# JaronTu/Multimodal_MVD_Seg

Hardware: AMD Instinct MI355X
Metric: train-step samples/sec on 4-modality 128^3 patches (PlainConvUNet 3d_fullres, fp32) (higher is better)
Workload: dtype f32; 1 GPU; BASELINE configs[1]: PlainConvUNet 3d_fullres 6 stages 31.2M params, 4x128x128x128 patch, 5 classes, fp32, DC+CE deep supervision, SGD-Nesterov+clip; per_gpu_batch=2, global_batch=2, parallelism=dp1, step_launch=one hipGraph replay per step (captured after 3 eager steps)

## Files before the change

multimodal_mvd_seg_amd/csrc/conv_mfma.hip:

```cpp
#include <stdlib.h>
#include <type_traits>

#include "common.h"
#include "conv_geom.h"

namespace mvd {

typedef float f32x16 __attribute__((ext_vector_type(16)));

struct FwdTile {
    int ED, EH, EW, nslots;
    int min_off[3];
    int ntd, nth, ntw;
    int K;
    int toff[27];
    int dbg;
};

__device__ __forceinline__ void store_tile32(const FwdGeom &g, const f32x16 &acc, float bv, int n, int od, int ohb, int ow0,
                                             int k, int hh, int S, int split, int Ktot, float *__restrict__ part,
                                             float *__restrict__ y1, float *__restrict__ y2) {
    const int owl = ow0 + 4 * hh;
    if (S > 1) {
        float *pl = part + (size_t)(4 * hh) * Ktot + k;
// ... 360 lines not shown
        if (c0 < g.C1) {
            src = a1; Cs = g.C1; cofs = c0;
        } else {
            src = a2; Cs = g.C2; cofs = c0 - g.C1;
        }
        load_w(cc, 0);
        __syncthreads();
        for (int base = 0; base < XR; base += XB) {
            float4 v[XB];
#pragma unroll
            for (int u = 0; u < XB; u++) {
                const int idx = (base + u) * 256 + tid;
                v[u] = make_float4(0.f, 0.f, 0.f, 0.f);
                if (base + u < XR && idx < nx && !(tg.dbg & 1)) {
                    const int slot = idx >> 3;
                    const int ez = (slot * tg.magHW) >> 16, rem = slot - ez * EHW;
                    const int ey = (rem * tg.magW) >> 16, ex = rem - ey * tg.EW;
                    const int id = iz0 + ez, ih = iy0 + ey, iw = ix0 + ex;
                    if (id >= 0 && id < g.Di && ih >= 0 && ih < g.Hi && iw >= 0 && iw < g.Wi)
                        v[u] = *reinterpret_cast<const float4 *>(
                            src + ((((size_t)n * g.Di + id) * g.Hi + ih) * g.Wi + iw) * Cs + cofs + (tid & 7) * 4);
                }
            }
#pragma unroll
            for (int u = 0; u < XB; u++) {
                const int idx = (base + u) * 256 + tid;
                if (base + u < XR) *reinterpret_cast<float4 *>(Xs + (size_t)(idx >> 3) * XS + (idx & 7) * 4) = v[u];
            }
        }
        for (int gi = 0; gi < ngroups; gi++) {
            store_w(gi & 1);
            __syncthreads();
            if (gi + 1 < ngroups) load_w(cc, gi + 1);
            if (!(tg.dbg & 2)) {
                const float *wb_ = Wsm + (size_t)(gi & 1) * WBUF;
#pragma unroll
                for (int tl = 0; tl < TG; tl++) {
                    const int t = gi * TG + tl;
                    if (t < g.ntaps) {
                        const int to = __builtin_amdgcn_readlane(toff_l, t);
                        float4 af[MT][4], bf[NT][4];
#pragma unroll
                        for (int m = 0; m < MT; m++) {
                            const float4 *pa = reinterpret_cast<const float4 *>(Xs + (size_t)(sbase[m] + to) * XS + h * 16);
#pragma unroll
                            for (int e = 0; e < 4; e++) af[m][e] = pa[e];
                        }
#pragma unroll
                        for (int q = 0; q < NT; q++) {
                            const float4 *pb = reinterpret_cast<const float4 *>(wb_ + ((size_t)(tl * 2 + h) * KT + q * 32 + i) * WS);
#pragma unroll
                            for (int e = 0; e < 4; e++) bf[q][e] = pb[e];
                        }
#pragma unroll
                        for (int e = 0; e < 4; e++) {
#pragma unroll
                            for (int c4 = 0; c4 < 4; c4++)
#pragma unroll
                                for (int m = 0; m < MT; m++)
#pragma unroll
                                    for (int q = 0; q < NT; q++) {
                                        const float avv = c4 == 0 ? af[m][e].x : (c4 == 1 ? af[m][e].y : (c4 == 2 ? af[m][e].z : af[m][e].w));
                                        const float bvv = c4 == 0 ? bf[q][e].x : (c4 == 1 ? bf[q][e].y : (c4 == 2 ? bf[q][e].z : bf[q][e].w));
                                        acc[m][q] = __builtin_amdgcn_mfma_f32_32x32x2f32(avv, bvv, acc[m][q], 0, 0, 0);
                                    }
                        }
                    }
                }
            }
        }
    }
    const int od = od0 + wave;
    if (od >= g.Do) return;
#pragma unroll
    for (int m = 0; m < MT; m++)
#pragma unroll
        for (int q = 0; q < NT; q++) {
            const int k = kb * KT + q * 32 + i;
            const float bv = settled((bias && tg.S == 1) ? bias[k] : 0.f);
            store_tile32(g, acc[m][q], bv, n, od, oh0 + 4 * m, ow0, k, h, tg.S, split, tg.K, part, y1, y2);
        }
}

constexpr int SXR = 12;
constexpr int SXB = 6;
__global__ __launch_bounds__(512, 1) void k_fwd32s(const FwdGeom g, const Fwd32Tile tg, const float *__restrict__ a1,
                                                   const float *__restrict__ a2, const float *__restrict__ w,
                                                   const float *__restrict__ bias, float *__restrict__ y1,
                                                   float *__restrict__ y2, float *__restrict__ stats) {
    extern __shared__ __attribute__((aligned(16))) float Xs[];
    constexpr int XS = 36;
    const int tid = threadIdx.x, lane = tid & 63;
    const int wave = __builtin_amdgcn_readfirstlane(tid >> 6);
    const int i = lane & 31, h = lane >> 5;
    const int per_xcd = (tg.nitems + 7) >> 3;
    const int item = (int)(blockIdx.x & 7) * per_xcd + (int)(blockIdx.x >> 3);
    if (item >= tg.nitems) return;
    unsigned r_ = (unsigned)item;
    const int kb = (int)(r_ % (unsigned)tg.nkb); r_ /= (unsigned)tg.nkb;
    const int tw_ = (int)(r_ % (unsigned)tg.ntw); r_ /= (unsigned)tg.ntw;
    const int th_ = (int)(r_ % (unsigned)tg.nth); r_ /= (unsigned)tg.nth;
    const int td_ = (int)(r_ % (unsigned)tg.ntd);
    const int n = (int)(r_ / (unsigned)tg.ntd);

    const int C = g.C1 + g.C2;
    const int nch = C >> 5;
    const int EHW = tg.EH * tg.EW;
    const int nx = tg.nslots * 8;
    const int od0 = td_ * 2, oh0 = th_ * 4, ow0 = tw_ * 8;
    const int iz0 = od0 * 2 + tg.min_off[0], iy0 = oh0 * 2 + tg.min_off[1], ix0 = ow0 * 2 + tg.min_off[2];
    const int dl = wave & 1, kh = (wave >> 1) & 1, tap_half = wave >> 2;
    const int tb = tap_half ? 14 : 0, nt = tap_half ? g.ntaps - 14 : 14;
    const int sbase = ((2 * dl) * tg.EH + 2 * (i >> 3)) * tg.EW + 2 * (i & 7);
    const float4 *xlane = reinterpret_cast<const float4 *>(Xs + (size_t)sbase * XS + h * 16);
    const int kcol = kb * 64 + kh * 32 + i;
    const float *wlane = w + (((size_t)h * tg.K + kcol) << 4);
    const size_t wtap = (size_t)2 * tg.K * 16;

    const bool fastst = tg.EH == 9 && tg.EW == 17 && tg.nslots == 765;
    const int r3 = tid / 136, rem = tid - r3 * 136;
    const int sx = rem >> 3, part = rem & 7;
    const bool st_act = tid < 408;
    const int iw = ix0 + sx;
    const bool okw = st_act && iw >= 0 && iw < g.Wi;
    bool okr[3];
#pragma unroll
    for (int v = 0; v < 3; v++) {
        const int ih = iy0 + r3 + 3 * v;
        okr[v] = okw && ih >= 0 && ih < g.Hi;
    }
    float4 *lds_st = reinterpret_cast<float4 *>(Xs + (size_t)(r3 * 17 + sx) * XS + part * 4);

    f32x16 acc;
#pragma unroll
    for (int r = 0; r < 16; r++) acc[r] = 0.f;
    const int lt = lane < g.ntaps ? lane : g.ntaps - 1;
    const int toff_l = tg.toff[lt < 27 ? lt : 26], wt_l = g.wt[lt < 27 ? lt : 26];

    for (int cc = 0; cc < nch; cc++) {
        const int c0 = cc * 32;
        const float *src;
        int Cs, cofs;
        if (c0 < g.C1) {
            src = a1; Cs = g.C1; cofs = c0;
        } else {
            src = a2; Cs = g.C2; cofs = c0 - g.C1;
        }
        const float *wc = wlane + (size_t)cc * g.T * wtap;
        float4 wb[4][4];
#pragma unroll
        for (int u = 0; u < 3; u++)
#pragma unroll
            for (int e = 0; e < 4; e++)
                wb[u][e] = *reinterpret_cast<const float4 *>(wc + (size_t)__builtin_amdgcn_readlane(wt_l, tb + u) * wtap + e * 4);
        __syncthreads();
        if (fastst) {
            const unsigned off0 = (unsigned)(((iy0 + r3) * g.Wi + iw) * Cs + cofs + part * 4) << 2;
            const unsigned drow = (unsigned)(3 * g.Wi * Cs) << 2;
            float4 v[15];
#pragma unroll
            for (int pl = 0; pl < 5; pl++) {
                const int id = iz0 + pl;
                const bool inpl = id >= 0 && id < g.Di;
                const float *plane = src + ((size_t)n * g.Di + (inpl ? id : 0)) * g.Hi * g.Wi * Cs;
                const __amdgpu_buffer_rsrc_t rp =
                    __builtin_amdgcn_make_buffer_rsrc(const_cast<float *>(plane), 0, inpl ? 0x7fffffff : 0, 0x00020000);
#pragma unroll
                for (int r = 0; r < 3; r++) {
                    const unsigned o = okr[r] ? off0 + (unsigned)r * drow : 0xffffffffu;
                    v[pl * 3 + r] = __builtin_bit_cast(float4, __builtin_amdgcn_raw_buffer_load_b128(rp, (int)o, 0, 0));
                }
            }
#pragma unroll
            for (int pq = 0; pq < 15; pq++)
                if (st_act) lds_st[((pq / 3) * 9 + 3 * (pq % 3)) * 17 * (XS / 4)] = v[pq];
        } else {
            int tid_ = tid;
            asm volatile("" : "+v"(tid_));
            for (int base = 0; base < SXR; base += SXB) {
                float4 v[SXB];
#pragma unroll
                for (int q = 0; q < SXB; q++) {
                    const int idx = (base + q) * 512 + tid_;
                    v[q] = make_float4(0.f, 0.f, 0.f, 0.f);
                    if (idx < nx) {
                        const int slot = idx >> 3;
                        const int ez = slot / EHW, rem2 = slot - ez * EHW;
                        const int ey = (rem2 * tg.magW) >> 16, ex = rem2 - ey * tg.EW;
                        const int id = iz0 + ez, ih = iy0 + ey, iw2 = ix0 + ex;
                        if (id >= 0 && id < g.Di && ih >= 0 && ih < g.Hi && iw2 >= 0 && iw2 < g.Wi)
                            v[q] = *reinterpret_cast<const float4 *>(
                                src + ((((size_t)n * g.Di + id) * g.Hi + ih) * g.Wi + iw2) * Cs + cofs + (tid_ & 7) * 4);
                    }
                }
#pragma unroll
                for (int q = 0; q < SXB; q++) {
                    const int idx = (base + q) * 512 + tid_;
                    if (idx < nx) *reinterpret_cast<float4 *>(Xs + (size_t)(idx >> 3) * XS + (idx & 7) * 4) = v[q];
                }
            }
        }
        __syncthreads();
        float4 af[2][4];
        {
            const float4 *pa = xlane + (size_t)__builtin_amdgcn_readlane(toff_l, tb) * (XS / 4);
#pragma unroll
            for (int e = 0; e < 4; e++) af[0][e] = pa[e];
        }
        for (int s0 = 0; s0 < nt; s0 += 4) {
#pragma unroll
            for (int u = 0; u < 4; u++) {
                const int sidx = s0 + u;
                if (sidx < nt) {
                    const int t = tb + sidx;
                    const int tn = sidx + 3 < nt ? t + 3 : tb + nt - 1;
#pragma unroll
                    for (int e = 0; e < 4; e++)
                        wb[(u + 3) & 3][e] =
                            *reinterpret_cast<const float4 *>(wc + (size_t)__builtin_amdgcn_readlane(wt_l, tn) * wtap + e * 4);
                    const float4 *pa = xlane + (size_t)__builtin_amdgcn_readlane(toff_l, sidx + 1 < nt ? t + 1 : tb + nt - 1) * (XS / 4);
#pragma unroll
                    for (int e = 0; e < 4; e++) af[(u + 1) & 1][e] = pa[e];
#pragma unroll
                    for (int e = 0; e < 4; e++) {
                        acc = __builtin_amdgcn_mfma_f32_32x32x2f32(af[u & 1][e].x, wb[u][e].x, acc, 0, 0, 0);
                        acc = __builtin_amdgcn_mfma_f32_32x32x2f32(af[u & 1][e].y, wb[u][e].y, acc, 0, 0, 0);
                        acc = __builtin_amdgcn_mfma_f32_32x32x2f32(af[u & 1][e].z, wb[u][e].z, acc, 0, 0, 0);
                        acc = __builtin_amdgcn_mfma_f32_32x32x2f32(af[u & 1][e].w, wb[u][e].w, acc, 0, 0, 0);
                    }
                    __builtin_amdgcn_sched_barrier(0);
                }
            }
        }
    }
    __syncthreads();
    if (tap_half) {
        float *xo = Xs + (size_t)(wave & 3) * 1024 + lane;
#pragma unroll
        for (int r = 0; r < 16; r++) xo[r * 64] = acc[r];
    }
    __syncthreads();
    if (tap_half) return;
    {
        const float *xi = Xs + (size_t)wave * 1024 + lane;
#pragma unroll
        for (int r = 0; r < 16; r++) acc[r] += xi[r * 64];
    }
    const int od = od0 + dl;
    const float bv = settled(bias ? bias[kcol] : 0.f);
    if (stats) {
        const size_t tl = ((size_t)(td_ * 2 + dl) * tg.nth + th_) * tg.ntw + tw_;
        float *so = stats + (((size_t)n * tg.ntd * 2 * tg.nth * tg.ntw + tl) * tg.K) * 2;
        float sa = 0.f, sq = 0.f;
        if (od < g.Do) {
#pragma unroll
            for (int r = 0; r < 16; r++) {
                const int row = (r & 3) + 8 * (r >> 2) + 4 * h;
                const int oh = oh0 + (row >> 3), ow = ow0 + (row & 7);
                if (oh < g.Ho && ow < g.Wo) {
                    const float val = acc[r] + bv;
                    sa += val;
                    sq += val * val;
                }
            }
        }
        sa += __shfl_xor(sa, 32);
        sq += __shfl_xor(sq, 32);
        if (h == 0) *reinterpret_cast<float2 *>(so + (size_t)kcol * 2) = make_float2(sa, sq);
    }
    if (od >= g.Do) return;
#pragma unroll
    for (int r = 0; r < 16; r++) {
        const int row = (r & 3) + 8 * (r >> 2) + 4 * h;
        const int oh = oh0 + (row >> 3), ow = ow0 + (row & 7);
        if (oh < g.Ho && ow < g.Wo) {
            const size_t ov = (((size_t)n * g.Dy + od) * g.Hy + oh) * g.Wy + ow;
            const float val = acc[r] + bv;
            if (kcol < g.K1)
                y1[ov * g.K1 + kcol] = val;
            else
                y2[ov * g.K2 + (kcol - g.K1)] = val;
        }
    }
}

struct Dg2Tile {
    int ntd, nth, ntw, ncb, nitems, C;
    int acc;
};
__global__ __launch_bounds__(512, 2) void k_dgrad32s(const FwdGeom g, const Dg2Tile tg, const float *__restrict__ dy,
                                                     const float *__restrict__ wb, float *__restrict__ dx) {
    __shared__ __attribute__((aligned(16))) float Xs[135 * 36];
    constexpr int XS = 36;
    const int tid = threadIdx.x, lane = tid & 63;
    const int wave = __builtin_amdgcn_readfirstlane(tid >> 6);
    const int i = lane & 31, h = lane >> 5;
    const int per_xcd = (tg.nitems + 7) >> 3;
    const int item = (int)(blockIdx.x & 7) * per_xcd + (int)(blockIdx.x >> 3);
    if (item >= tg.nitems) return;
    unsigned r_ = (unsigned)item;
    const int cb = (int)(r_ % (unsigned)tg.ncb); r_ /= (unsigned)tg.ncb;
    const int tw_ = (int)(r_ % (unsigned)tg.ntw); r_ /= (unsigned)tg.ntw;
    const int th_ = (int)(r_ % (unsigned)tg.nth); r_ /= (unsigned)tg.nth;
    const int td_ = (int)(r_ % (unsigned)tg.ntd);
    const int n = (int)(r_ / (unsigned)tg.ntd);
    const int K = g.C1, C = tg.C;
    const int nch = K >> 5;
    const int oz0 = td_ * 2, oy0 = th_ * 4, ox0 = tw_ * 8;
    const int ccol = cb * 32 + i;
    const float *wlane = wb + (((size_t)h * C + ccol) << 4);
    const size_t wtap = (size_t)2 * C * 16;

    f32x16 acc[2];
#pragma unroll
    for (int m = 0; m < 2; m++)
#pragma unroll
        for (int r = 0; r < 16; r++) acc[m][r] = 0.f;

    for (int kk = 0; kk < nch; kk++) {
        __syncthreads();
        {
            const __amdgpu_buffer_rsrc_t rdy = __builtin_amdgcn_make_buffer_rsrc(
                const_cast<float *>(dy + (size_t)n * g.Di * g.Hi * g.Wi * K + kk * 32), 0, 0x7fffffff, 0x00020000);
            float4 v[3];
#pragma unroll
            for (int u = 0; u < 3; u++) {
                const int idx = tid + u * 512;
                const int slot = idx >> 3, part = idx & 7;
                const int ez = slot / 45, rem = slot - ez * 45;
                const int ey = rem / 9, ex = rem - ey * 9;
                const int oz = oz0 + ez, oy = oy0 + ey, ox = ox0 + ex;
                const bool ok = idx < 135 * 8 && oz < g.Di && oy < g.Hi && ox < g.Wi;
                const unsigned o = ok ? (unsigned)(((oz * g.Hi + oy) * g.Wi + ox) * K + part * 4) * 4u : 0xffffffffu;
                v[u] = __builtin_bit_cast(float4, __builtin_amdgcn_raw_buffer_load_b128(rdy, (int)o, 0, 0));
            }
#pragma unroll
            for (int u = 0; u < 3; u++) {
                const int idx = tid + u * 512;
                if (idx < 135 * 8) *reinterpret_cast<float4 *>(Xs + (size_t)(idx >> 3) * XS + (idx & 7) * 4) = v[u];
            }
        }
        __syncthreads();
        const float *wc = wlane + (size_t)kk * 27 * wtap;
#pragma unroll
        for (int m = 0; m < 2; m++) {
            const int q = m ? 7 - wave : wave;
            const int pz = q >> 2, py = (q >> 1) & 1, px = q & 1;
            const float4 *xm = reinterpret_cast<const float4 *>(Xs + (size_t)((m * 5 + (i >> 3)) * 9 + (i & 7)) * XS + h * 16);
            const int ntq = 1 << (pz + py + px);
            auto tap_of = [&](int j, int &t, int &so) {
                const int bz = pz ? (j >> (py + px)) & 1 : 0, by = py ? (j >> px) & 1 : 0, bx = px ? j & 1 : 0;
                const int tz = pz ? (bz ? 2 : 0) : 1, ty = py ? (by ? 2 : 0) : 1, tx = px ? (bx ? 2 : 0) : 1;
                const int dz = (pz && !bz) ? 1 : 0, dyy = (py && !by) ? 1 : 0, dxx = (px && !bx) ? 1 : 0;
                t = (tz * 3 + ty) * 3 + tx;
                so = (dz * 5 + dyy) * 9 + dxx;
            };
            float4 wv[2][4];
            int t0, so0;
            tap_of(0, t0, so0);
#pragma unroll
            for (int e = 0; e < 4; e++) wv[0][e] = *reinterpret_cast<const float4 *>(wc + (size_t)t0 * wtap + e * 4);
            for (int j = 0; j < ntq; j += 2) {
#pragma unroll
                for (int u = 0; u < 2; u++) {
                    if (j + u < ntq) {
                        int t, so, tn, son;
                        tap_of(j + u, t, so);
                        tap_of(j + u + 1 < ntq ? j + u + 1 : j + u, tn, son);
#pragma unroll
                        for (int e = 0; e < 4; e++)
                            wv[(u + 1) & 1][e] = *reinterpret_cast<const float4 *>(wc + (size_t)tn * wtap + e * 4);
                        float4 af[4];
#pragma unroll
                        for (int e = 0; e < 4; e++) af[e] = xm[so * (XS / 4) + e];
#pragma unroll
                        for (int e = 0; e < 4; e++) {
                            acc[m] = __builtin_amdgcn_mfma_f32_32x32x2f32(af[e].x, wv[u][e].x, acc[m], 0, 0, 0);
                            acc[m] = __builtin_amdgcn_mfma_f32_32x32x2f32(af[e].y, wv[u][e].y, acc[m], 0, 0, 0);
                            acc[m] = __builtin_amdgcn_mfma_f32_32x32x2f32(af[e].z, wv[u][e].z, acc[m], 0, 0, 0);
                            acc[m] = __builtin_amdgcn_mfma_f32_32x32x2f32(af[e].w, wv[u][e].w, acc[m], 0, 0, 0);
                        }
                    }
                }
            }
        }
    }
    float *xl = dx + (size_t)(2 * 4 * h) * C + ccol;
#pragma unroll
    for (int m = 0; m < 2; m++) {
        const int q = m ? 7 - wave : wave;
        const int pz = q >> 2, py = (q >> 1) & 1, px = q & 1;
        const int iz = 2 * (oz0 + m) + pz;
#pragma unroll
        for (int r = 0; r < 16; r++) {
            const int iy = 2 * (oy0 + (r >> 2)) + py, ixu = 2 * (ox0 + (r & 3)) + px;
            const size_t uo = ((((size_t)n * g.Dy + iz) * g.Hy + iy) * g.Wy + ixu) * C;
            if (iz < g.Dy && iy < g.Hy && ixu + 8 * h < g.Wy) xl[uo] = tg.acc ? xl[uo] + acc[m][r] : acc[m][r];
        }
    }
}

int dgrad32s(int N, int D, int H, int W, int C, int K, int Do, int Ho, int Wo, const float *dy, const float *wb, float *dx,
             hipStream_t s, int accumulate) {
    if (C % 32 || K % 32 || (((uintptr_t)dy | (uintptr_t)wb) & 15)) return -1;
    if ((long)Do * Ho * Wo * K * 4 >= (1L << 31)) return -1;
    FwdGeom g;
    memset(&g, 0, sizeof(g));
    g.N = N;
    g.Di = Do; g.Hi = Ho; g.Wi = Wo;
    g.Dy = D; g.Hy = H; g.Wy = W;
    g.C1 = K;
    Dg2Tile tg;
    tg.ntd = (Do + 1) / 2; tg.nth = (Ho + 3) / 4; tg.ntw = (Wo + 7) / 8;
    tg.ncb = C / 32;
    tg.C = C;
    tg.acc = accumulate;
    const long nitems = (long)N * tg.ntd * tg.nth * tg.ntw * tg.ncb;
    if (nitems > (1L << 30)) return -1;
    tg.nitems = (int)nitems;
    const unsigned grid = (unsigned)(((nitems + 7) / 8) * 8);
    hipLaunchKernelGGL(k_dgrad32s, dim3(grid), dim3(512), 0, s, g, tg, dy, wb, dx);
    return check_launch("conv dgrad (stride 2, fused parity classes)");
}

static int num_cus();
static int launch_fwd32s(const FwdGeom &g, const float *a1, const float *a2, const float *w, const float *bias, float *y1,
                         float *y2, hipStream_t s, float *stats, long stats_tiles, int *stats_done, long *plan) {
    const int K = g.K1 + g.K2;
    Fwd32Tile tg;
    memset(&tg, 0, sizeof(tg));
    int mn[3] = {127, 127, 127}, mx[3] = {-127, -127, -127};
    for (int t = 0; t < g.ntaps; t++)
        for (int a = 0; a < 3; a++) {
            if (g.off[t][a] < mn[a]) mn[a] = g.off[t][a];
            if (g.off[t][a] > mx[a]) mx[a] = g.off[t][a];
        }
    const int T3[3] = {2, 4, 8};
    int E[3];
    for (int a = 0; a < 3; a++) {
        E[a] = (T3[a] - 1) * 2 + (mx[a] - mn[a]) + 1;
        tg.min_off[a] = mn[a];
    }
    tg.EH = E[1]; tg.EW = E[2];
    tg.nslots = E[0] * E[1] * E[2];
    if (tg.nslots > SXR * 64 || g.ntaps != 27) return -1;
    int m = (1 << 16) / tg.EW + 1;
    for (int nn = 0; nn < tg.EH * tg.EW; nn++)
        if (((nn * m) >> 16) != nn / tg.EW) return -1;
    tg.magW = m;
    for (int t = 0; t < g.ntaps; t++)
        tg.toff[t] = ((g.off[t][0] - mn[0]) * tg.EH + (g.off[t][1] - mn[1])) * tg.EW + (g.off[t][2] - mn[2]);
    tg.ntd = (g.Do + 1) / 2;
    tg.nth = (g.Ho + 3) / 4;
    tg.ntw = (g.Wo + 7) / 8;
    tg.nkb = K / 64;
    tg.K = K;
    const long nitems = (long)g.N * tg.ntd * tg.nth * tg.ntw * tg.nkb;
    if (nitems > (1L << 30)) return -1;
    tg.nitems = (int)nitems;
    const long my_tiles = (long)tg.ntd * 2 * tg.nth * tg.ntw;
    if (plan) {
        *plan = my_tiles;
        return 0;
    }
    float *st = (stats && stats_done && stats_tiles == my_tiles) ? stats : nullptr;
    const size_t lds = (size_t)tg.nslots * 36 * sizeof(float);
    static PerDeviceFlag cfgd;
    if (!cfgd()) {
        if (hipFuncSetAttribute(reinterpret_cast<const void *>(k_fwd32s), hipFuncAttributeMaxDynamicSharedMemorySize,
                                (int)LDS_LIMIT) != hipSuccess) {
            set_error("conv fwd (stride 2): cannot raise the dynamic LDS limit");
            return 1;
        }
        cfgd() = true;
    }
    const unsigned grid = (unsigned)(((nitems + 7) / 8) * 8);
    hipLaunchKernelGGL(k_fwd32s, dim3(grid), dim3(512), lds, s, g, tg, a1, a2, w, bias, y1, y2, st);
    if (check_launch("conv fwd (stride 2, CK=32)")) return 1;
    if (st) *stats_done = 1;
    return 0;
}

static int num_cus() {
    static int n = 0;
    if (!n) {
        hipDeviceProp_t p;
        int dev = 0;
        if (hipGetDevice(&dev) == hipSuccess && hipGetDeviceProperties(&p, dev) == hipSuccess) n = p.multiProcessorCount;
        if (n <= 0) n = 256;
    }
    return n;
}

static int split_for(const void *ws, size_t ws_bytes, long wgs, int nch, size_t out_elems, int nkb) {
    int S = 1;
    if (ws && wgs < 256 && nch >= 4) {
        long want = 512 / wgs;
        if (want > MAX_SPLIT) want = MAX_SPLIT;
        if (want > nch / 2) want = nch / 2;
        while (want > 1 && (size_t)want * out_elems * sizeof(float) > ws_bytes) want--;
        if (want > 1 && (long)nkb * want <= 65535) S = (int)want;
    }
    return S;
}

static int run_split_reduce(const FwdGeom &g, const float *part, const float *bias, float *y1, float *y2, int S,
                            size_t out_elems, hipStream_t s) {
    long blocks = cdiv((long)out_elems, 256);
    if (blocks > 2048) blocks = 2048;
    hipLaunchKernelGGL(k_split_reduce, dim3(blocks), dim3(256), 0, s, g, part, bias, y1, y2, S);
    return check_launch("conv fwd split reduce");
}

template <int NT, int TG>
static int launch_fwd32(const FwdGeom &g, Fwd32Tile &tg, const float *a1, const float *a2, const float *w,
                        const float *bias, float *y1, float *y2, void *ws, size_t ws_bytes, hipStream_t s) {
    auto kern = k_fwd32<NT, TG>;
    constexpr int XR = 12;
    const size_t lds = ((size_t)XR * 32 * 36 + 2 * (size_t)TG * 2 * (32 * NT) * 20) * 4;
    static PerDeviceFlag configured;
    if (!configured()) {
        if (hipFuncSetAttribute(reinterpret_cast<const void *>(kern), hipFuncAttributeMaxDynamicSharedMemorySize,
                                (int)LDS_LIMIT) != hipSuccess) {
            set_error("conv fwd32 (mfma): cannot raise the dynamic LDS limit");
            return 1;
        }
        configured() = true;
    }
    const int K = g.K1 + g.K2;
    tg.nkb = K / (32 * NT);
    const long tiles = (long)tg.ntd * tg.nth * tg.ntw;
    const size_t out_elems = (size_t)g.N * g.Do * g.Ho * g.Wo * K;
    tg.S = split_for(ws, ws_bytes, tiles * tg.nkb * g.N, (g.C1 + g.C2) / 32, out_elems, tg.nkb);
    const long nitems = tiles * tg.nkb * tg.S * g.N;
    if (nitems > (1L << 30)) return -1;
    tg.nitems = (int)nitems;
    const long grid = ((nitems + 7) / 8) * 8;
    float *part = reinterpret_cast<float *>(ws);
    hipLaunchKernelGGL(kern, dim3((unsigned)grid), dim3(256), lds, s, g, tg, a1, a2, w, bias, y1, y2, part);
    if (check_launch("conv fwd32 (mfma)")) return 1;
    if (tg.S > 1) return run_split_reduce(g, part, bias, y1, y2, tg.S, out_elems, s);
    return 0;
}

template <int CK, int NT, int MT, bool L32>
static int launch_fwd(const FwdGeom &g, FwdTile &tg, size_t lds, const float *a1, const float *a2, const float *w,
                      const float *bias, float *y1, float *y2, void *ws, size_t ws_bytes, hipStream_t s, float *stats,
                      long stats_tiles, int *stats_done, long *plan) {
    const long my_tiles = (long)tg.ntd * 4 * tg.nth * tg.ntw;
    if (plan) {
        *plan = my_tiles;
        return 0;
    }
    float *st = (stats && stats_done && stats_tiles == my_tiles) ? stats : nullptr;
    auto kern = k_fwd_mfma<CK, NT, MT, L32>;
    static size_t configured = 0;
    if (lds > configured) {
        if (hipFuncSetAttribute(reinterpret_cast<const void *>(kern), hipFuncAttributeMaxDynamicSharedMemorySize,
                                (int)LDS_LIMIT) != hipSuccess) {
            set_error("conv fwd (mfma): cannot raise the dynamic LDS limit");
            return 1;
        }
        configured = LDS_LIMIT;
    }
    const int K = g.K1 + g.K2;
    const int nkb = K / (32 * NT);
    const long tiles = (long)tg.ntd * tg.nth * tg.ntw;
    const size_t out_elems = (size_t)g.N * g.Do * g.Ho * g.Wo * K;
    const int S = st ? 1 : split_for(ws, ws_bytes, tiles * nkb * g.N, (g.C1 + g.C2) / CK, out_elems, nkb);
    dim3 grid((unsigned)tiles, nkb * S, g.N);
    float *part = reinterpret_cast<float *>(ws);
    hipLaunchKernelGGL(kern, grid, dim3(256), lds, s, g, tg, a1, a2, w, bias, y1, y2, S, part, st);
    if (check_launch("conv fwd (mfma)")) return 1;
    if (S > 1) return run_split_reduce(g, part, bias, y1, y2, S, out_elems, s);
    if (st) *stats_done = 1;
    return 0;
}

int fwd_mfma(const FwdGeom &g, const float *a1, const float *a2, const float *w, const float *bias, float *y1, float *y2,
             void *ws, size_t ws_bytes, hipStream_t s, float *stats, long stats_tiles, int *stats_done, long *plan) {
    if (plan) *plan = 0;
    if (stats_done) *stats_done = 0;
    if (g.K2 != 0 || g.so[0] != 1 || g.so[1] != 1 || g.so[2] != 1 || g.oo[0] || g.oo[1] || g.oo[2]) {
        stats = nullptr;
        if (plan) return 0;
    }
    const int C = g.C1 + g.C2, K = g.K1 + g.K2;
    const int LCK = wl_ck(C);
    if (LCK == 0 || g.ntaps < 1 || g.ntaps > 27) return -1;
    if (g.C1 % LCK != 0 || g.C2 % LCK != 0) return -1;
    if (K % 32 != 0 || g.K1 % 32 != 0 || g.K2 % 32 != 0) return -1;
    if (g.N > 65535 || K / 32 > 65535) return -1;
    if (((uintptr_t)a1 | (uintptr_t)a2 | (uintptr_t)w) & 15) return -1;
    static int dbg = -1;
    if (dbg < 0) dbg = getenv("MVD_CONV_DBG") ? atoi(getenv("MVD_CONV_DBG")) : 0;
    int mn[3] = {127, 127, 127}, mx[3] = {-127, -127, -127};
    for (int t = 0; t < g.ntaps; t++)
        for (int a = 0; a < 3; a++) {
            if (g.off[t][a] < mn[a]) mn[a] = g.off[t][a];
            if (g.off[t][a] > mx[a]) mx[a] = g.off[t][a];
        }
    const bool unit_stride = g.sa[0] == 1 && g.sa[1] == 1 && g.sa[2] == 1;
    if (LCK == 32 && unit_stride && !(dbg & 4)) {
        static int nt_rule = -1;
        if (nt_rule < 0) nt_rule = getenv("MVD_CONV_NT") ? atoi(getenv("MVD_CONV_NT")) : 1;
        const long wg64 = (long)g.N * ((g.Do + 3) / 4) * ((g.Ho + 3) / 4) * ((g.Wo + 7) / 8) * (K / 64);
        const int NT = (K % 64 == 0 && !(nt_rule == 1 && wg64 < 128)) ? 2 : 1;
        Fwd32Tile t32;
        memset(&t32, 0, sizeof(t32));
        t32.dbg = dbg;
        const int T3[3] = {4, 4, 8};
        int E[3];
        for (int a = 0; a < 3; a++) {
            E[a] = (T3[a] - 1) + (mx[a] - mn[a]) + 1;
            t32.min_off[a] = mn[a];
        }
        t32.EH = E[1]; t32.EW = E[2];
        t32.nslots = E[0] * E[1] * E[2];
        auto magic = [](int d, int nmax) -> int {
            int m = (1 << 16) / d + 1;
            for (int n = 0; n < nmax; n++)
                if (((n * m) >> 16) != n / d) return -1;
            return m;
        };
        t32.magHW = magic(t32.EH * t32.EW, t32.nslots);
        t32.magW = magic(t32.EW, t32.EH * t32.EW);
        if (t32.nslots <= 12 * 32 && t32.magHW > 0 && t32.magW > 0) {
            for (int t = 0; t < g.ntaps; t++)
                t32.toff[t] = ((g.off[t][0] - mn[0]) * t32.EH + (g.off[t][1] - mn[1])) * t32.EW + (g.off[t][2] - mn[2]);
            t32.ntd = (g.Do + 3) / 4;
            t32.nth = (g.Ho + 3) / 4;
            t32.ntw = (g.Wo + 7) / 8;
            t32.K = K;
            if (plan) return 0;
            if (NT == 2) return launch_fwd32<2, 1>(g, t32, a1, a2, w, bias, y1, y2, ws, ws_bytes, s);
            return launch_fwd32<1, 2>(g, t32, a1, a2, w, bias, y1, y2, ws, ws_bytes, s);
        }
    }
    if (LCK == 32 && g.sa[0] == 2 && g.sa[1] == 2 && g.sa[2] == 2 && g.ntaps == 27 && g.T == 27 && K % 64 == 0 &&
        g.K1 % 64 == 0 && g.so[0] == 1 && g.so[1] == 1 && g.so[2] == 1 && g.oo[0] == 0 && g.oo[1] == 0 && g.oo[2] == 0 &&
        !(dbg & 8)) {
        const long items = (long)g.N * ((g.Do + 1) / 2) * ((g.Ho + 3) / 4) * ((g.Wo + 7) / 8) * (K / 64);
        if (items >= 256) {
            int r = launch_fwd32s(g, a1, a2, w, bias, y1, y2, s, stats, stats_tiles, stats_done, plan);
            if (r >= 0) return r;
        }
    }
    const int CK = LCK == 32 ? 8 : LCK;
    FwdTile tg;
    memset(&tg, 0, sizeof(tg));
    tg.dbg = dbg;
    tg.K = K;
    const int cand[3][2] = {{2, 2}, {2, 1}, {1, 1}};
    for (int ci = 0; ci < 3; ci++) {
        const int MT = cand[ci][0], NT = cand[ci][1];
        if (K % (32 * NT) != 0) continue;
        const int T3[3] = {4, 4 * MT, 8};
        int E[3];
        for (int a = 0; a < 3; a++) {
            E[a] = (T3[a] - 1) * g.sa[a] + (mx[a] - mn[a]) + 1;
            tg.min_off[a] = mn[a];
        }
        tg.ED = E[0]; tg.EH = E[1]; tg.EW = E[2];
        tg.nslots = E[0] * E[1] * E[2];
        const size_t lds = ((size_t)tg.nslots * CK + (size_t)g.ntaps * 2 * (32 * NT) * (CK / 2)) * 4 + 64 * 4;
        const bool fits2 = lds <= LDS_LIMIT / 2;
        const bool last = (ci == 2);
        if (!fits2 && !(last && lds <= LDS_LIMIT)) {
            if (!last) continue;
            return -1;
        }
        for (int t = 0; t < g.ntaps; t++)
            tg.toff[t] = ((g.off[t][0] - mn[0]) * tg.EH + (g.off[t][1] - mn[1])) * tg.EW + (g.off[t][2] - mn[2]);
        tg.ntd = (g.Do + 3) / 4;
        tg.nth = (g.Ho + 4 * MT - 1) / (4 * MT);
        tg.ntw = (g.Wo + 7) / 8;
#define MVD_FWD_DISPATCH(CKV, L32V)                                                                                      \
    {                                                                                                                    \
        if (MT == 2 && NT == 2) return launch_fwd<CKV, 2, 2, L32V>(g, tg, lds, a1, a2, w, bias, y1, y2, ws, ws_bytes, s, stats, stats_tiles, stats_done, plan); \
        if (MT == 2 && NT == 1) return launch_fwd<CKV, 1, 2, L32V>(g, tg, lds, a1, a2, w, bias, y1, y2, ws, ws_bytes, s, stats, stats_tiles, stats_done, plan); \
        return launch_fwd<CKV, 1, 1, L32V>(g, tg, lds, a1, a2, w, bias, y1, y2, ws, ws_bytes, s, stats, stats_tiles, stats_done, plan); \
    }
        if (LCK == 32) MVD_FWD_DISPATCH(8, true)
        else if (CK == 8) MVD_FWD_DISPATCH(8, false)
        else MVD_FWD_DISPATCH(4, false)
#undef MVD_FWD_DISPATCH
    }
    return -1;
}

struct WgTile {
    int TD, TH, TW, lTH, lTW;
    int EAh, EAw, nslotsA, minA[3];
    int EBh, EBw, nslotsB, minB[3];
    int magAw, magAhw, magBw, magBhw;
    int ntd, nth, ntw, nsplit, nkb;
    int ntiles;
    int toffA[27], toffB[27];
    int dbg;
};

template <int TPW, int NA, int NB, int SH>
__global__ __launch_bounds__(512, 1) void k_wgrad_mfma(const WgradGeom g, const WgTile tg, const float *__restrict__ a1,
                                                       const float *__restrict__ a2, const float *__restrict__ b,
                                                       float *__restrict__ partial, float *__restrict__ pbias) {
    extern __shared__ __attribute__((aligned(16))) float lds[];
    float *As = lds;
    float *Bs = lds + (size_t)NA * 2048;
    const int tid = threadIdx.x, lane = tid & 63;
    const int wave8 = __builtin_amdgcn_readfirstlane(tid >> 6);
    const int wave = wave8 & 3, grp = wave8 >> 2;
    const int i = lane & 31, h = lane >> 5;
    const int cb = blockIdx.y / tg.nkb, kb = blockIdx.y % tg.nkb;
    const int split = blockIdx.x;
    const int C = g.C1 + g.C2, K = g.K;

    int ta[TPW], tb[TPW];
#pragma unroll
    for (int j = 0; j < TPW; j++) {
        ta[j] = tb[j] = 0;
#pragma unroll
        for (int t = 0; t < 27; t++)
            if (t == wave + 4 * j && t < g.ntaps) {
                ta[j] = tg.toffA[t];
                tb[j] = tg.toffB[t];
            }
// ... 1742 lines not shown
```

Before: 61.41 samples/s.

## Shrink stride-2 fwd conv tiles and double-buffer dgrad LDS staging

The stride-2 forward conv kernel now covers one output depth plane per 256-thread block instead of two planes per 512-thread block. That shrinks the LDS halo to 459 slots, allows two blocks per CU, and remaps the fast-path staging loads and the stats write for out-of-range planes. The stride-2 dgrad kernel gains a double-buffered dy tile in LDS, prefetch of the next chunk and a rotating weight prefetch via buffer loads. Its per-wave tap lists are balanced across the two output planes and it targets 4 blocks per CU. The fwd32s dispatch threshold is also relaxed. This trades more halo re-reads and more blocks for better occupancy and latency hiding, at the risk of register pressure under the tighter launch bounds.

```diff
diff --git a/multimodal_mvd_seg_amd/csrc/conv_mfma.hip b/multimodal_mvd_seg_amd/csrc/conv_mfma.hip
--- a/multimodal_mvd_seg_amd/csrc/conv_mfma.hip
+++ b/multimodal_mvd_seg_amd/csrc/conv_mfma.hip
@@ -466,9 +466,9 @@
         }
 }
 
-constexpr int SXR = 12;
-constexpr int SXB = 6;
-__global__ __launch_bounds__(512, 1) void k_fwd32s(const FwdGeom g, const Fwd32Tile tg, const float *__restrict__ a1,
+constexpr int SXR = 15;
+constexpr int SXB = 5;
+__global__ __launch_bounds__(256, 2) void k_fwd32s(const FwdGeom g, const Fwd32Tile tg, const float *__restrict__ a1,
                                                    const float *__restrict__ a2, const float *__restrict__ w,
                                                    const float *__restrict__ bias, float *__restrict__ y1,
                                                    float *__restrict__ y2, float *__restrict__ stats) {
@@ -484,36 +484,42 @@
     const int kb = (int)(r_ % (unsigned)tg.nkb); r_ /= (unsigned)tg.nkb;
     const int tw_ = (int)(r_ % (unsigned)tg.ntw); r_ /= (unsigned)tg.ntw;
     const int th_ = (int)(r_ % (unsigned)tg.nth); r_ /= (unsigned)tg.nth;
-    const int td_ = (int)(r_ % (unsigned)tg.ntd);
-    const int n = (int)(r_ / (unsigned)tg.ntd);
+    const int npl = tg.ntd * 2;
+    const int od = (int)(r_ % (unsigned)npl);
+    const int n = (int)(r_ / (unsigned)npl);
 
     const int C = g.C1 + g.C2;
     const int nch = C >> 5;
     const int EHW = tg.EH * tg.EW;
     const int nx = tg.nslots * 8;
-    const int od0 = td_ * 2, oh0 = th_ * 4, ow0 = tw_ * 8;
-    const int iz0 = od0 * 2 + tg.min_off[0], iy0 = oh0 * 2 + tg.min_off[1], ix0 = ow0 * 2 + tg.min_off[2];
-    const int dl = wave & 1, kh = (wave >> 1) & 1, tap_half = wave >> 2;
+    const int oh0 = th_ * 4, ow0 = tw_ * 8;
+    const int iz0 = od * 2 + tg.min_off[0], iy0 = oh0 * 2 + tg.min_off[1], ix0 = ow0 * 2 + tg.min_off[2];
+    const int kh = wave & 1, tap_half = wave >> 1;
     const int tb = tap_half ? 14 : 0, nt = tap_half ? g.ntaps - 14 : 14;
-    const int sbase = ((2 * dl) * tg.EH + 2 * (i >> 3)) * tg.EW + 2 * (i & 7);
+    const int sbase = (2 * (i >> 3)) * tg.EW + 2 * (i & 7);
     const float4 *xlane = reinterpret_cast<const float4 *>(Xs + (size_t)sbase * XS + h * 16);
     const int kcol = kb * 64 + kh * 32 + i;
+    float *so = stats ? stats + (((size_t)n * npl * tg.nth * tg.ntw + ((size_t)od * tg.nth + th_) * tg.ntw + tw_) * tg.K) * 2
+                      : nullptr;
+    if (od >= g.Do) {
+        if (so && !tap_half && h == 0) *reinterpret_cast<float2 *>(so + (size_t)kcol * 2) = make_float2(0.f, 0.f);
+        return;
+    }
     const float *wlane = w + (((size_t)h * tg.K + kcol) << 4);
     const size_t wtap = (size_t)2 * tg.K * 16;
 
-    const bool fastst = tg.EH == 9 && tg.EW == 17 && tg.nslots == 765;
-    const int r3 = tid / 136, rem = tid - r3 * 136;
-    const int sx = rem >> 3, part = rem & 7;
-    const bool st_act = tid < 408;
-    const int iw = ix0 + sx;
-    const bool okw = st_act && iw >= 0 && iw < g.Wi;
-    bool okr[3];
-#pragma unroll
-    for (int v = 0; v < 3; v++) {
-        const int ih = iy0 + r3 + 3 * v;
-        okr[v] = okw && ih >= 0 && ih < g.Hi;
-    }
-    float4 *lds_st = reinterpret_cast<float4 *>(Xs + (size_t)(r3 * 17 + sx) * XS + part * 4);
+    const bool fastst = tg.EH == 9 && tg.EW == 17 && tg.nslots == 459;
+    const int ssl = tid >> 3, part = tid & 7;
+    int spos[5];
+#pragma unroll
+    for (int u = 0; u < 5; u++) {
+        const int t17 = (32 * u) % 17 + ssl;
+        const int kq = (t17 >= 17 ? 1 : 0) + (t17 >= 34 ? 1 : 0);
+        const int ih = iy0 + (32 * u) / 17 + kq, iw = ix0 + t17 - 17 * kq;
+        const bool ok = (u < 4 || ssl < 25) && ih >= 0 && ih < g.Hi && iw >= 0 && iw < g.Wi;
+        spos[u] = ok ? ih * g.Wi + iw : -1;
+    }
+    float4 *lds_st = reinterpret_cast<float4 *>(Xs + (size_t)ssl * XS + part * 4);
 
     f32x16 acc;
 #pragma unroll
@@ -539,25 +545,25 @@
                 wb[u][e] = *reinterpret_cast<const float4 *>(wc + (size_t)__builtin_amdgcn_readlane(wt_l, tb + u) * wtap + e * 4);
         __syncthreads();
         if (fastst) {
-            const unsigned off0 = (unsigned)(((iy0 + r3) * g.Wi + iw) * Cs + cofs + part * 4) << 2;
-            const unsigned drow = (unsigned)(3 * g.Wi * Cs) << 2;
+            unsigned offs[5];
+#pragma unroll
+            for (int u = 0; u < 5; u++)
+                offs[u] = spos[u] >= 0 ? (unsigned)(spos[u] * Cs + cofs + part * 4) << 2 : 0xffffffffu;
             float4 v[15];
 #pragma unroll
-            for (int pl = 0; pl < 5; pl++) {
+            for (int pl = 0; pl < 3; pl++) {
                 const int id = iz0 + pl;
                 const bool inpl = id >= 0 && id < g.Di;
                 const float *plane = src + ((size_t)n * g.Di + (inpl ? id : 0)) * g.Hi * g.Wi * Cs;
                 const __amdgpu_buffer_rsrc_t rp =
                     __builtin_amdgcn_make_buffer_rsrc(const_cast<float *>(plane), 0, inpl ? 0x7fffffff : 0, 0x00020000);
 #pragma unroll
-                for (int r = 0; r < 3; r++) {
-                    const unsigned o = okr[r] ? off0 + (unsigned)r * drow : 0xffffffffu;
-                    v[pl * 3 + r] = __builtin_bit_cast(float4, __builtin_amdgcn_raw_buffer_load_b128(rp, (int)o, 0, 0));
-                }
+                for (int u = 0; u < 5; u++)
+                    v[pl * 5 + u] = __builtin_bit_cast(float4, __builtin_amdgcn_raw_buffer_load_b128(rp, (int)offs[u], 0, 0));
             }
 #pragma unroll
             for (int pq = 0; pq < 15; pq++)
-                if (st_act) lds_st[((pq / 3) * 9 + 3 * (pq % 3)) * 17 * (XS / 4)] = v[pq];
+                if (pq % 5 < 4 || ssl < 25) lds_st[((pq / 5) * 153 + 32 * (pq % 5)) * (XS / 4)] = v[pq];
         } else {
             int tid_ = tid;
             asm volatile("" : "+v"(tid_));
@@ -565,7 +571,7 @@
                 float4 v[SXB];
 #pragma unroll
                 for (int q = 0; q < SXB; q++) {
-                    const int idx = (base + q) * 512 + tid_;
+                    const int idx = (base + q) * 256 + tid_;
                     v[q] = make_float4(0.f, 0.f, 0.f, 0.f);
                     if (idx < nx) {
                         const int slot = idx >> 3;
@@ -579,7 +585,7 @@
                 }
 #pragma unroll
                 for (int q = 0; q < SXB; q++) {
-                    const int idx = (base + q) * 512 + tid_;
+                    const int idx = (base + q) * 256 + tid_;
                     if (idx < nx) *reinterpret_cast<float4 *>(Xs + (size_t)(idx >> 3) * XS + (idx & 7) * 4) = v[q];
                 }
             }
@@ -619,40 +625,34 @@
     }
     __syncthreads();
     if (tap_half) {
-        float *xo = Xs + (size_t)(wave & 3) * 1024 + lane;
+        float *xo = Xs + (size_t)kh * 1024 + lane;
 #pragma unroll
         for (int r = 0; r < 16; r++) xo[r * 64] = acc[r];
     }
     __syncthreads();
     if (tap_half) return;
     {
-        const float *xi = Xs + (size_t)wave * 1024 + lane;
+        const float *xi = Xs + (size_t)kh * 1024 + lane;
 #pragma unroll
         for (int r = 0; r < 16; r++) acc[r] += xi[r * 64];
     }
-    const int od = od0 + dl;
     const float bv = settled(bias ? bias[kcol] : 0.f);
-    if (stats) {
-        const size_t tl = ((size_t)(td_ * 2 + dl) * tg.nth + th_) * tg.ntw + tw_;
-        float *so = stats + (((size_t)n * tg.ntd * 2 * tg.nth * tg.ntw + tl) * tg.K) * 2;
+    if (so) {
         float sa = 0.f, sq = 0.f;
-        if (od < g.Do) {
-#pragma unroll
-            for (int r = 0; r < 16; r++) {
-                const int row = (r & 3) + 8 * (r >> 2) + 4 * h;
-                const int oh = oh0 + (row >> 3), ow = ow0 + (row & 7);
-                if (oh < g.Ho && ow < g.Wo) {
-                    const float val = acc[r] + bv;
-                    sa += val;
-                    sq += val * val;
-                }
+#pragma unroll
+        for (int r = 0; r < 16; r++) {
+            const int row = (r & 3) + 8 * (r >> 2) + 4 * h;
+            const int oh = oh0 + (row >> 3), ow = ow0 + (row & 7);
+            if (oh < g.Ho && ow < g.Wo) {
+                const float val = acc[r] + bv;
+                sa += val;
+                sq += val * val;
             }
         }
         sa += __shfl_xor(sa, 32);
         sq += __shfl_xor(sq, 32);
         if (h == 0) *reinterpret_cast<float2 *>(so + (size_t)kcol * 2) = make_float2(sa, sq);
     }
-    if (od >= g.Do) return;
 #pragma unroll
     for (int r = 0; r < 16; r++) {
         const int row = (r & 3) + 8 * (r >> 2) + 4 * h;
@@ -668,14 +668,18 @@
     }
 }
 
+template <int V>
+struct IntC {
+    static constexpr int value = V;
+};
 struct Dg2Tile {
     int ntd, nth, ntw, ncb, nitems, C;
     int acc;
 };
-__global__ __launch_bounds__(512, 2) void k_dgrad32s(const FwdGeom g, const Dg2Tile tg, const float *__restrict__ dy,
+__global__ __launch_bounds__(512, 4) void k_dgrad32s(const FwdGeom g, const Dg2Tile tg, const float *__restrict__ dy,
                                                      const float *__restrict__ wb, float *__restrict__ dx) {
-    __shared__ __attribute__((aligned(16))) float Xs[135 * 36];
-    constexpr int XS = 36;
+    constexpr int XS = 36, IMG = 135 * XS;
+    __shared__ __attribute__((aligned(16))) float Xs[2 * IMG];
     const int tid = threadIdx.x, lane = tid & 63;
     const int wave = __builtin_amdgcn_readfirstlane(tid >> 6);
     const int i = lane & 31, h = lane >> 5;
@@ -692,8 +696,9 @@
     const int nch = K >> 5;
     const int oz0 = td_ * 2, oy0 = th_ * 4, ox0 = tw_ * 8;
     const int ccol = cb * 32 + i;
-    const float *wlane = wb + (((size_t)h * C + ccol) << 4);
-    const size_t wtap = (size_t)2 * C * 16;
+    const __amdgpu_buffer_rsrc_t rw = __builtin_amdgcn_make_buffer_rsrc(const_cast<float *>(wb), 0, 0x7fffffff, 0x00020000);
+    const int wlane = ((h * C + ccol) << 4) * 4;
+    const int wtap = 2 * C * 16 * 4;
 
     f32x16 acc[2];
 #pragma unroll
@@ -701,77 +706,118 @@
 #pragma unroll
         for (int r = 0; r < 16; r++) acc[m][r] = 0.f;
 
-    for (int kk = 0; kk < nch; kk++) {
+    const int pcw = __builtin_popcount((unsigned)wave);
+    const int sm = pcw <= 1 ? 0 : 1, ns = (pcw == 0 || pcw == 3) ? 1 : 2, nt = ns + 8 / ns;
+    int ts_l;
+    {
+        const int jl = lane < nt ? lane : nt - 1;
+        const int m = jl < ns ? sm : 1 - sm;
+        const int j = jl < ns ? jl : jl - ns;
+        const int q = m ? 7 - wave : wave;
+        const int pz = q >> 2, py = (q >> 1) & 1, px = q & 1;
+        const int bz = pz ? (j >> (py + px)) & 1 : 0, by = py ? (j >> px) & 1 : 0, bx = px ? j & 1 : 0;
+        const int tz = pz ? (bz ? 2 : 0) : 1, ty = py ? (by ? 2 : 0) : 1, tx = px ? (bx ? 2 : 0) : 1;
+        const int dz = (pz && !bz) ? 1 : 0, dyy = (py && !by) ? 1 : 0, dxx = (px && !bx) ? 1 : 0;
+        ts_l = ((((m + dz) * 5 + dyy) * 9 + dxx) << 8) | ((tz * 3 + ty) * 3 + tx);
+    }
+    const float4 *xm = reinterpret_cast<const float4 *>(Xs + (size_t)((i >> 3) * 9 + (i & 7)) * XS + h * 16);
+
+    auto dy_off = [&](int idx) -> unsigned {
+        const int slot = idx >> 3, part = idx & 7;
+        const int ez = slot / 45, rem = slot - ez * 45;
+        const int ey = rem / 9, ex = rem - ey * 9;
+        const int oz = oz0 + ez, oy = oy0 + ey, ox = ox0 + ex;
+        const bool ok = idx < 135 * 8 && oz < g.Di && oy < g.Hi && ox < g.Wi;
+        return ok ? (unsigned)(((oz * g.Hi + oy) * g.Wi + ox) * K + part * 4) * 4u : 0xffffffffu;
+    };
+    unsigned dyo[2];
+#pragma unroll
+    for (int u = 0; u < 2; u++) dyo[u] = dy_off(tid + u * 512);
+    const float *dyn = dy + (size_t)n * g.Di * g.Hi * g.Wi * K;
+    auto dy_rsrc = [&](int kk) {
+        const bool in = kk < nch;
+        return __builtin_amdgcn_make_buffer_rsrc(const_cast<float *>(dyn + (in ? kk : 0) * 32), 0, in ? 0x7fffffff : 0,
+                                                 0x00020000);
+    };
+    float4 v[2];
+    auto load_dy = [&](int kk) {
+        const __amdgpu_buffer_rsrc_t rdy = dy_rsrc(kk);
+#pragma unroll
+        for (int u = 0; u < 2; u++)
+            v[u] = __builtin_bit_cast(float4, __builtin_amdgcn_raw_buffer_load_b128(rdy, (int)dyo[u], 0, 0));
+    };
+    auto store_dy = [&](int kk) {
+        float *img = Xs + (size_t)(kk & 1) * IMG;
+#pragma unroll
+        for (int u = 0; u < 2; u++) {
+            const int idx = tid + u * 512;
+            *reinterpret_cast<float4 *>(img + (size_t)(idx >> 3) * XS + (idx & 7) * 4) = v[u];
+        }
+        if (wave == 1) {
+            const int idx = 1024 + lane;
+            const float4 t = __builtin_bit_cast(float4, __builtin_amdgcn_raw_buffer_load_b128(dy_rsrc(kk), (int)dy_off(idx), 0, 0));
+            if (idx < 135 * 8) *reinterpret_cast<float4 *>(img + (size_t)(idx >> 3) * XS + (idx & 7) * 4) = t;
+        }
+    };
+    auto chunks = [&](auto ntc) {
+        constexpr int NT = decltype(ntc)::value, NS = NT == 9 ? 1 : 2;
+        float4 wv[3][4], af[2][4];
+        load_dy(0);
+    #pragma unroll
+        for (int u = 0; u < 2; u++)
+    #pragma unroll
+            for (int e = 0; e < 4; e++)
+                wv[u][e] = __builtin_bit_cast(float4, __builtin_amdgcn_raw_buffer_load_b128(
+                    rw, wlane + e * 16, (__builtin_amdgcn_readlane(ts_l, u) & 255) * wtap, 0));
+        store_dy(0);
         __syncthreads();
-        {
-            const __amdgpu_buffer_rsrc_t rdy = __builtin_amdgcn_make_buffer_rsrc(
-                const_cast<float *>(dy + (size_t)n * g.Di * g.Hi * g.Wi * K + kk * 32), 0, 0x7fffffff, 0x00020000);
-            float4 v[3];
-#pragma unroll
-            for (int u = 0; u < 3; u++) {
-                const int idx = tid + u * 512;
-                const int slot = idx >> 3, part = idx & 7;
-                const int ez = slot / 45, rem = slot - ez * 45;
-                const int ey = rem / 9, ex = rem - ey * 9;
-                const int oz = oz0 + ez, oy = oy0 + ey, ox = ox0 + ex;
-                const bool ok = idx < 135 * 8 && oz < g.Di && oy < g.Hi && ox < g.Wi;
-                const unsigned o = ok ? (unsigned)(((oz * g.Hi + oy) * g.Wi + ox) * K + part * 4) * 4u : 0xffffffffu;
-                v[u] = __builtin_bit_cast(float4, __builtin_amdgcn_raw_buffer_load_b128(rdy, (int)o, 0, 0));
-            }
-#pragma unroll
-            for (int u = 0; u < 3; u++) {
-                const int idx = tid + u * 512;
-                if (idx < 135 * 8) *reinterpret_cast<float4 *>(Xs + (size_t)(idx >> 3) * XS + (idx & 7) * 4) = v[u];
-            }
-        }
-        __syncthreads();
-        const float *wc = wlane + (size_t)kk * 27 * wtap;
-#pragma unroll
-        for (int m = 0; m < 2; m++) {
-            const int q = m ? 7 - wave : wave;
-            const int pz = q >> 2, py = (q >> 1) & 1, px = q & 1;
-            const float4 *xm = reinterpret_cast<const float4 *>(Xs + (size_t)((m * 5 + (i >> 3)) * 9 + (i & 7)) * XS + h * 16);
-            const int ntq = 1 << (pz + py + px);
-            auto tap_of = [&](int j, int &t, int &so) {
-                const int bz = pz ? (j >> (py + px)) & 1 : 0, by = py ? (j >> px) & 1 : 0, bx = px ? j & 1 : 0;
-                const int tz = pz ? (bz ? 2 : 0) : 1, ty = py ? (by ? 2 : 0) : 1, tx = px ? (bx ? 2 : 0) : 1;
-                const int dz = (pz && !bz) ? 1 : 0, dyy = (py && !by) ? 1 : 0, dxx = (px && !bx) ? 1 : 0;
-                t = (tz * 3 + ty) * 3 + tx;
-                so = (dz * 5 + dyy) * 9 + dxx;
-            };
-            float4 wv[2][4];
-            int t0, so0;
-            tap_of(0, t0, so0);
-#pragma unroll
-            for (int e = 0; e < 4; e++) wv[0][e] = *reinterpret_cast<const float4 *>(wc + (size_t)t0 * wtap + e * 4);
-            for (int j = 0; j < ntq; j += 2) {
-#pragma unroll
-                for (int u = 0; u < 2; u++) {
-                    if (j + u < ntq) {
-                        int t, so, tn, son;
-                        tap_of(j + u, t, so);
-                        tap_of(j + u + 1 < ntq ? j + u + 1 : j + u, tn, son);
-#pragma unroll
-                        for (int e = 0; e < 4; e++)
-                            wv[(u + 1) & 1][e] = *reinterpret_cast<const float4 *>(wc + (size_t)tn * wtap + e * 4);
-                        float4 af[4];
-#pragma unroll
-                        for (int e = 0; e < 4; e++) af[e] = xm[so * (XS / 4) + e];
-#pragma unroll
-                        for (int e = 0; e < 4; e++) {
-                            acc[m] = __builtin_amdgcn_mfma_f32_32x32x2f32(af[e].x, wv[u][e].x, acc[m], 0, 0, 0);
-                            acc[m] = __builtin_amdgcn_mfma_f32_32x32x2f32(af[e].y, wv[u][e].y, acc[m], 0, 0, 0);
-                            acc[m] = __builtin_amdgcn_mfma_f32_32x32x2f32(af[e].z, wv[u][e].z, acc[m], 0, 0, 0);
-                            acc[m] = __builtin_amdgcn_mfma_f32_32x32x2f32(af[e].w, wv[u][e].w, acc[m], 0, 0, 0);
-                        }
-                    }
-                }
-            }
-        }
-    }
-    float *xl = dx + (size_t)(2 * 4 * h) * C + ccol;
-#pragma unroll
-    for (int m = 0; m < 2; m++) {
+        for (int kk = 0; kk < nch; kk++) {
+            const int wc = kk * 27 * wtap;
+            const int wnx = kk + 1 < nch ? wc + 27 * wtap : wc;
+            load_dy(kk + 1);
+            const float4 *xb = xm + (size_t)(kk & 1) * (IMG / 4);
+            {
+                const float4 *pa = xb + (size_t)(__builtin_amdgcn_readlane(ts_l, 0) >> 8) * (XS / 4);
+#pragma unroll
+                for (int e = 0; e < 4; e++) af[0][e] = pa[e];
+            }
+#pragma unroll
+            for (int j = 0; j < NT; j++) {
+                const int wsrc = (j + 2 < NT ? wc : wnx) + (__builtin_amdgcn_readlane(ts_l, (j + 2) % NT) & 255) * wtap;
+#pragma unroll
+                for (int e = 0; e < 4; e++)
+                    wv[(j + 2) % 3][e] =
+                        __builtin_bit_cast(float4, __builtin_amdgcn_raw_buffer_load_b128(rw, wlane + e * 16, wsrc, 0));
+                if (j + 1 < NT) {
+                    const float4 *pa = xb + (size_t)(__builtin_amdgcn_readlane(ts_l, j + 1) >> 8) * (XS / 4);
+#pragma unroll
+                    for (int e = 0; e < 4; e++) af[(j + 1) & 1][e] = pa[e];
+                }
+                const int a = j < NS ? 0 : 1;
+#pragma unroll
+                for (int e = 0; e < 4; e++) {
+                    acc[a] = __builtin_amdgcn_mfma_f32_32x32x2f32(af[j & 1][e].x, wv[j % 3][e].x, acc[a], 0, 0, 0);
+                    acc[a] = __builtin_amdgcn_mfma_f32_32x32x2f32(af[j & 1][e].y, wv[j % 3][e].y, acc[a], 0, 0, 0);
+                    acc[a] = __builtin_amdgcn_mfma_f32_32x32x2f32(af[j & 1][e].z, wv[j % 3][e].z, acc[a], 0, 0, 0);
+                    acc[a] = __builtin_amdgcn_mfma_f32_32x32x2f32(af[j & 1][e].w, wv[j % 3][e].w, acc[a], 0, 0, 0);
+                }
+                __builtin_amdgcn_sched_barrier(0);
+            }
+            store_dy(kk + 1);
+            __syncthreads();
+        }
+    };
+    if (nt == 9)
+        chunks(IntC<9>{});
+    else
+        chunks(IntC<6>{});
+    int tid_ = tid;
+    asm volatile("" : "+v"(tid_));
+    const int h_ = (tid_ >> 5) & 1;
+    float *xl = dx + (size_t)(2 * 4 * h_) * C + cb * 32 + (tid_ & 31);
+#pragma unroll
+    for (int a = 0; a < 2; a++) {
+        const int m = a ? 1 - sm : sm;
         const int q = m ? 7 - wave : wave;
         const int pz = q >> 2, py = (q >> 1) & 1, px = q & 1;
         const int iz = 2 * (oz0 + m) + pz;
@@ -779,7 +825,7 @@
         for (int r = 0; r < 16; r++) {
             const int iy = 2 * (oy0 + (r >> 2)) + py, ixu = 2 * (ox0 + (r & 3)) + px;
             const size_t uo = ((((size_t)n * g.Dy + iz) * g.Hy + iy) * g.Wy + ixu) * C;
-            if (iz < g.Dy && iy < g.Hy && ixu + 8 * h < g.Wy) xl[uo] = tg.acc ? xl[uo] + acc[m][r] : acc[m][r];
+            if (iz < g.Dy && iy < g.Hy && ixu + 8 * h_ < g.Wy) xl[uo] = tg.acc ? xl[uo] + acc[a][r] : acc[a][r];
         }
     }
 }
@@ -788,6 +834,7 @@
              hipStream_t s, int accumulate) {
     if (C % 32 || K % 32 || (((uintptr_t)dy | (uintptr_t)wb) & 15)) return -1;
     if ((long)Do * Ho * Wo * K * 4 >= (1L << 31)) return -1;
+    if ((long)K * 27 * 2 * C * 16 * 4 >= (1L << 31)) return -1;
     FwdGeom g;
     memset(&g, 0, sizeof(g));
     g.N = N;
@@ -819,7 +866,7 @@
             if (g.off[t][a] < mn[a]) mn[a] = g.off[t][a];
             if (g.off[t][a] > mx[a]) mx[a] = g.off[t][a];
         }
-    const int T3[3] = {2, 4, 8};
+    const int T3[3] = {1, 4, 8};
     int E[3];
     for (int a = 0; a < 3; a++) {
         E[a] = (T3[a] - 1) * 2 + (mx[a] - mn[a]) + 1;
@@ -827,7 +874,7 @@
     }
     tg.EH = E[1]; tg.EW = E[2];
     tg.nslots = E[0] * E[1] * E[2];
-    if (tg.nslots > SXR * 64 || g.ntaps != 27) return -1;
+    if (tg.nslots > SXR * 32 || tg.nslots < 57 || g.ntaps != 27) return -1;
     int m = (1 << 16) / tg.EW + 1;
     for (int nn = 0; nn < tg.EH * tg.EW; nn++)
         if (((nn * m) >> 16) != nn / tg.EW) return -1;
@@ -839,7 +886,7 @@
     tg.ntw = (g.Wo + 7) / 8;
     tg.nkb = K / 64;
     tg.K = K;
-    const long nitems = (long)g.N * tg.ntd * tg.nth * tg.ntw * tg.nkb;
+    const long nitems = (long)g.N * tg.ntd * 2 * tg.nth * tg.ntw * tg.nkb;
     if (nitems > (1L << 30)) return -1;
     tg.nitems = (int)nitems;
     const long my_tiles = (long)tg.ntd * 2 * tg.nth * tg.ntw;
@@ -859,7 +906,7 @@
         cfgd() = true;
     }
     const unsigned grid = (unsigned)(((nitems + 7) / 8) * 8);
-    hipLaunchKernelGGL(k_fwd32s, dim3(grid), dim3(512), lds, s, g, tg, a1, a2, w, bias, y1, y2, st);
+    hipLaunchKernelGGL(k_fwd32s, dim3(grid), dim3(256), lds, s, g, tg, a1, a2, w, bias, y1, y2, st);
     if (check_launch("conv fwd (stride 2, CK=32)")) return 1;
     if (st) *stats_done = 1;
     return 0;
@@ -1024,8 +1071,8 @@
     if (LCK == 32 && g.sa[0] == 2 && g.sa[1] == 2 && g.sa[2] == 2 && g.ntaps == 27 && g.T == 27 && K % 64 == 0 &&
         g.K1 % 64 == 0 && g.so[0] == 1 && g.so[1] == 1 && g.so[2] == 1 && g.oo[0] == 0 && g.oo[1] == 0 && g.oo[2] == 0 &&
         !(dbg & 8)) {
-        const long items = (long)g.N * ((g.Do + 1) / 2) * ((g.Ho + 3) / 4) * ((g.Wo + 7) / 8) * (K / 64);
-        if (items >= 256) {
+        const long items = (long)g.Do * ((g.Ho + 3) / 4) * ((g.Wo + 7) / 8) * (K / 64);
+        if (items >= 128) {
             int r = launch_fwd32s(g, a1, a2, w, bias, y1, y2, s, stats, stats_tiles, stats_done, plan);
             if (r >= 0) return r;
         }
```

Result: no change. 61.89 samples/s, median of 6 (+0.8%).
